# RocketFlash/EmbeddingNet

Hardware: AMD Instinct MI355X
Metric: images/sec training (ResNet18, 224², triplet batch-hard) @ 1/2/4/8 GPU (higher is better)
Workload: dtype f32; 1 GPU; resnet18 224x224x3 synthetic U[0,1), 107-class P x K sampling, local batch 32x4=128 (139 resident batches cycled), E=256, margin 0.5, mining 'hardest' per local batch, radam, fp32 tensors (conv products on 16-bit MFMA from operand splits, fp32 accumulate: 3x3 stride-1 convs and their weight gradients, and the ResNets' other convs where both operands' ranges are known: two fp16 pieces + a per-tenso; global_batch=128, parallelism=dp1, active_triplets_min=192, dead_steps=0, resident_batches=139, step_mode=eager, mining=hardest

## Files before the change

### embeddingnet_amd/csrc/conv_patch.hip

```cpp
#include "gemm_engine.h"
#include "conv_geom.h"
#include "multi_tensor.h"
#include "../../include/embnet.h"

namespace embnet {
namespace patch {

typedef __attribute__((address_space(3))) void* lds_ptr;
__device__ __forceinline__ void dma16(__amdgpu_buffer_rsrc_t r, unsigned char* lds, unsigned voff, unsigned soff) {
  __builtin_amdgcn_raw_ptr_buffer_load_lds(r, (lds_ptr)lds, 16, (int)voff, (int)soff, 0, 0);
}

template <int BN_>
struct GeomP {
  static constexpr int BM = 256, BN = BN_, WAVES_M = 4, WAVES_N = 2, WTM = 64, WTN = BN_ / 2, TM = 2, TN = WTN / 32;
};

struct PatchParams {
  const unsigned short* xp;
  const unsigned short* wp;
  float* y; const float* bias; const float* residual; float* stats; int stats_rows; int relu;
  ConvGeom g; unsigned x_plane_bytes, w_plane_bytes;
  int PH, PW; FastDiv dPHW, dPW;
  int LR;
  int n_full, parts, cc_part, n_pieces, grid; float* ws;
  BnSums bn;
  const uint32_t* a_range; unsigned x32_bytes;
};

typedef const PatchParams __attribute__((address_space(4)))* kargp;
__device__ __forceinline__ kargp kargs() {
  kargp pp = (kargp)__builtin_amdgcn_kernarg_segment_ptr();
  asm volatile("" : "+s"(pp));
  return pp;
}

struct Item { int m0, n0, cc_b, cc_e, tile_m; float* part; };

template <int BN, int CCH = 16>
__device__ __forceinline__ Item work_item(int item, int n_mine) {
  kargp pp = kargs();
  const int b = blockIdx.x, NCC = pp->g.C / CCH, tiles_n = (pp->g.K + BN - 1) / BN;
  Item t; int id;
  if (item < n_mine) {
    id = b + item * pp->grid; t.cc_b = 0; t.cc_e = NCC; t.part = nullptr;
  }
  else {
    id = pp->n_full + b / pp->parts;
    t.cc_b = (b % pp->parts) * pp->cc_part; t.cc_e = min(NCC, t.cc_b + pp->cc_part);
    t.part = pp->ws + (long)b * (256 * BN);
  }
  t.tile_m = id / tiles_n; t.m0 = t.tile_m * 256; t.n0 = (id % tiles_n) * BN;
  return t;
}

__device__ __forceinline__ int padded_pos(int m) {
  kargp pp = kargs();
  FastDiv dOHW, dOW;
  dOHW.mul = pp->g.dOHW.mul; dOHW.shift = pp->g.dOHW.shift; dOHW.d = pp->g.dOHW.d;
  dOW.mul = pp->g.dOW.mul; dOW.shift = pp->g.dOW.shift; dOW.d = pp->g.dOW.d;
  uint32_t n, rem, oh, ow;
  dOHW.divmod((uint32_t)m, n, rem); dOW.divmod(rem, oh, ow);
  return (int)n * (pp->PH * pp->PW) + (int)oh * pp->PW + (int)ow;
}

template <class G, bool F16, int NP>
__device__ __forceinline__ void step_planes(const bf16x8 (&a)[G::TM][NP], const bf16x8 (&b)[G::TN][NP], f32x16 (&acc)[G::TM][G::TN]) {
  if constexpr (F16) {
    f16x8 ah[G::TM][2], bh[G::TN][2];
#pragma unroll
    for (int i = 0; i < G::TM; ++i) { ah[i][0] = __builtin_bit_cast(f16x8, a[i][0]); ah[i][1] = __builtin_bit_cast(f16x8, a[i][1]); }
#pragma unroll
    for (int i = 0; i < G::TN; ++i) { bh[i][0] = __builtin_bit_cast(f16x8, b[i][0]); bh[i][1] = __builtin_bit_cast(f16x8, b[i][1]); }
    mfma_step_h<G::TM, G::TN>(ah, bh, acc);
  } else {
    mfma_step3<G>(a, b, acc);
  }
}

template <class G, int BN, bool BNS, bool F16>
__device__ __forceinline__ void patch_epilogue(const PatchParams& p, const Item& cur, f32x16 (&acc)[G::TM][G::TN], int M, int K,
                                               int wave, int lane, int h, int wm, int wn) {
  constexpr int TM = G::TM, TN = G::TN;
  if (F16) {
    const float osx = p.a_range ? scale_pair(scale_exponent_of(__uint_as_float(*p.a_range))).y
                                : planes_scale_slot(p.xp, (long)(p.x_plane_bytes >> 1))[1];
    const float osw = planes_scale_slot(p.wp, (long)(p.w_plane_bytes >> 1))[1];
#pragma unroll
    for (int im = 0; im < TM; ++im)
#pragma unroll
      for (int in = 0; in < TN; ++in)
#pragma unroll
        for (int rr = 0; rr < 16; ++rr) acc[im][in][rr] = (acc[im][in][rr] * osw) * osx;
  }
  if (cur.part) {
    float* part = cur.part + (wm + 4 * h) * BN + wn + (lane & 31);
#pragma unroll
    for (int im = 0; im < TM; ++im)
#pragma unroll
      for (int in = 0; in < TN; ++in)
#pragma unroll
        for (int rr = 0; rr < 16; ++rr)
          part[(im * 32 + (rr & 3) + 8 * (rr >> 2)) * BN + in * 32] = acc[im][in][rr];
  } else {
    const bool inner = cur.m0 + 256 <= M && cur.n0 + BN <= K;
#pragma unroll
// ... 31 lines not shown
#pragma unroll
          for (int rr = 0; rr < 16; ++rr) {
            p.y[o0 + (long)((rr & 3) + 8 * (rr >> 2)) * K] = v[rr];
            if (BNS) {
              const float e = ev[BNS ? im : 0][rr], dz = act_grad(p.bn.act, fmaf(e, bsc, bsh), v[rr]);
              s1 += dz; s2 = fmaf(dz, (e - bmu) * brs, s2);
            } else { s1 += v[rr]; s2 = fmaf(v[rr], v[rr], s2); }
          }
        } else {
#pragma unroll
          for (int rr = 0; rr < 16; ++rr) {
            const int row = cur.m0 + wm + im * 32 + (rr & 3) + 8 * (rr >> 2) + 4 * h;
            if (row < M && cok) {
              const long o = o0 + (long)((rr & 3) + 8 * (rr >> 2)) * K;
              if (p.residual) v[rr] += p.residual[o];
              p.y[o] = v[rr];
              if (BNS) {
                const float e = ev[BNS ? im : 0][rr], dz = act_grad(p.bn.act, fmaf(e, bsc, bsh), v[rr]);
                s1 += dz; s2 = fmaf(dz, (e - bmu) * brs, s2);
              } else { s1 += v[rr]; s2 = fmaf(v[rr], v[rr], s2); }
            }
          }
        }
      }
      if (p.stats || bnm) {
        s1 += __shfl_xor(s1, 32, 64); s2 += __shfl_xor(s2, 32, 64);
        if (h == 0 && cok) {
          float* const dst = bnm ? p.bn.partial : p.stats;
          const long prow = (long)cur.tile_m * G::WAVES_M + wave / G::WAVES_N, P = bnm ? p.bn.rows : p.stats_rows;
          dst[(long)col * P + prow] = s1;
          dst[((long)K + col) * P + prow] = s2;
        }
      }
    }
  }

}

template <int BN, int R, int S, int TPS, int NBS, bool BNS = false, bool F16 = false, bool PIPE = false>
__global__ __launch_bounds__(640) void conv_patch_kernel(const PatchParams p) {
  using G = GeomP<BN>;
  constexpr int NP = F16 ? 2 : 3;
  constexpr int TM = G::TM, TN = G::TN, SPC = R * S / TPS, D = NBS - 1;
  constexpr int SBY = TPS * NP * BN * 32;
  constexpr int NBI = TPS * NP * (BN / 32);
  static_assert((R * S) % TPS == 0 && SPC >= 2, "steps per chunk");
  extern __shared__ __attribute__((aligned(16))) unsigned char smem[];
  const int tid = threadIdx.x, lane = tid & 63, h = lane >> 5;
  const int wave = __builtin_amdgcn_readfirstlane(tid >> 6);
  const int LR = p.LR, PLP = LR * 32, PB = NP * PLP;
  unsigned char* const bslot0 = smem + 2 * PB;
  const int b = blockIdx.x;
  const int n_mine = b < p.n_full ? (p.n_full - b + p.grid - 1) / p.grid : 0;
  const int n_items = n_mine + (b < p.n_pieces ? 1 : 0);
  if (n_items == 0) return;
  const int dhalf = (lane & 1) ^ ((lane >> 4) & 1);

  if (wave == 8) {
    const __amdgpu_buffer_rsrc_t wr = __builtin_amdgcn_make_buffer_rsrc(const_cast<unsigned short*>(p.wp), 0, 3u * p.w_plane_bytes, 0x00020000);
    const int K = p.g.K, NCC = p.g.C / 16;
    const unsigned wpb = p.w_plane_bytes;
    int it = 0; Item t = work_item<BN>(0, n_mine);
    int cc = t.cc_b, st = 0; bool live = true;
    unsigned rowoff[BN / 32];
    auto tile_rows = [&]() {
#pragma unroll
      for (int gb = 0; gb < BN / 32; ++gb) {
        const int row = t.n0 + gb * 32 + (lane >> 1);
        rowoff[gb] = row < K ? 32u * (unsigned)row + 16u * dhalf : OOB;
      }
    };
    tile_rows();
    auto issue = [&](int gs) {
      unsigned char* slot = bslot0 + (gs % NBS) * SBY;
#pragma unroll
      for (int tp = 0; tp < TPS; ++tp) {
        const int tap = st * TPS + tp, r = tap / S, s = tap % S;
        const unsigned so = 32u * (unsigned)(((r * NCC + cc) * S + s) * K);
#pragma unroll
        for (int q = 0; q < NP; ++q)
#pragma unroll
          for (int gb = 0; gb < BN / 32; ++gb)
            dma16(wr, slot + ((tp * NP + q) * BN + gb * 32) * 32, live ? rowoff[gb] : OOB, q * wpb + so);
      }
      if (live && ++st == SPC) {
        st = 0;
        if (++cc == t.cc_e) {
          if (++it < n_items) { t = work_item<BN>(it, n_mine); cc = t.cc_b; tile_rows(); } else live = false;
        }
      }
    };
    int total = 0;
    for (int i = 0; i < n_items; ++i) { const Item q = work_item<BN>(i, n_mine); total += (q.cc_e - q.cc_b) * SPC; }
    for (int gs = 0; gs < D; ++gs) issue(gs);
    for (int gs = 0; gs < total; ++gs) {
      asm volatile("s_waitcnt vmcnt(%0)" :: "n"((D - 1) * NBI) : "memory");
      __builtin_amdgcn_s_barrier();
      issue(gs + D);
    }
    asm volatile("s_waitcnt vmcnt(0)" ::: "memory");
    return;
  }
  if (wave == 9) {
    const __amdgpu_buffer_rsrc_t xr = __builtin_amdgcn_make_buffer_rsrc(const_cast<unsigned short*>(p.xp), 0, 3u * p.x_plane_bytes, 0x00020000);
    const int NG = LR / 32;
    const unsigned xpb = p.x_plane_bytes, chunk_bytes = 32u * (unsigned)(p.g.N * p.g.H * p.g.W);
    unsigned poff[16];
    auto tile_offsets = [&](const Item& t) {
      kargp pp = kargs();
      FastDiv dPHW, dPW;
      dPHW.mul = pp->dPHW.mul; dPHW.shift = pp->dPHW.shift; dPHW.d = pp->dPHW.d;
      dPW.mul = pp->dPW.mul; dPW.shift = pp->dPW.shift; dPW.d = pp->dPW.d;
      const int P0 = padded_pos(t.m0), N = pp->g.N, H = pp->g.H, W = pp->g.W, pt = pp->g.pad_t, pl = pp->g.pad_l;
#pragma unroll
      for (int gI = 0; gI < 16; ++gI) {
        const int idx = P0 + 32 * gI + (lane >> 1);
        uint32_t n, rem, py, px;
        dPHW.divmod((uint32_t)idx, n, rem); dPW.divmod(rem, py, px);
        const int ih = (int)py - pt, iw = (int)px - pl;
        const bool ok = gI < NG && (int)n < N && (unsigned)ih < (unsigned)H && (unsigned)iw < (unsigned)W;
        poff[gI] = ok ? 32u * (unsigned)(((int)n * H + ih) * W + iw) + 16u * dhalf : OOB;
      }
    };
    auto issue = [&](int cc, int gc) {
      unsigned char* buf = smem + (gc & 1) * PB;
#pragma unroll
      for (int q = 0; q < NP; ++q)
#pragma unroll
        for (int gI = 0; gI < 16; ++gI)
          if (gI < NG) dma16(xr, buf + q * PLP + gI * 1024, poff[gI], q * xpb + (unsigned)cc * chunk_bytes);
    };
    int it = 0; Item t = work_item<BN>(0, n_mine);
    int cc = t.cc_b; bool live = true;
    tile_offsets(t);
    auto advance = [&]() {
      if (++cc == t.cc_e) {
        if (++it < n_items) { t = work_item<BN>(it, n_mine); cc = t.cc_b; tile_offsets(t); } else live = false;
      }
    };
    issue(cc, 0); advance();
    int total_chunks = 0;
    for (int i = 0; i < n_items; ++i) { const Item q = work_item<BN>(i, n_mine); total_chunks += q.cc_e - q.cc_b; }
    for (int gc = 0; gc < total_chunks; ++gc) {
      asm volatile("s_waitcnt vmcnt(0)" ::: "memory");
      __builtin_amdgcn_s_barrier();
      if (live) { issue(cc, gc + 1); advance(); }
#pragma unroll 1
      for (int s2 = 1; s2 < SPC; ++s2) __builtin_amdgcn_s_barrier();
    }
    asm volatile("s_waitcnt vmcnt(0)" ::: "memory");
    return;
  }

  const int wm = (wave / G::WAVES_N) * G::WTM, wn = (wave % G::WAVES_N) * G::WTN;
  const int K = p.g.K, PW = p.PW, M = p.g.N * p.g.OH * p.g.OW;
  int gs = 0, gc = 0;
  f32x16 acc[TM][TN];
  for (int item = 0; item < n_items; ++item) {
    const Item cur = work_item<BN>(item, n_mine);
    int rowidx[TM];
    {
      const int P0 = padded_pos(cur.m0);
#pragma unroll
      for (int im = 0; im < TM; ++im) {
        const int m = cur.m0 + wm + im * 32 + (lane & 31);
        rowidx[im] = m < M ? padded_pos(m) - P0 : 0;
      }
    }
#pragma unroll
    for (int i = 0; i < TM; ++i)
#pragma unroll
      for (int j = 0; j < TN; ++j)
#pragma unroll
        for (int r = 0; r < 16; ++r) acc[i][j][r] = 0.f;
    for (int cc = cur.cc_b; cc < cur.cc_e; ++cc) {
      const unsigned char* pbuf = smem + (gc & 1) * PB;
      if constexpr (F16 && PIPE) {
        f16x8 fa[2][TM][2], fb[2][TN][2];
        auto load_a = [&](int tap, f16x8 (&a)[TM][2]) {
          const int r = tap / S, s2 = tap % S;
#pragma unroll
          for (int im = 0; im < TM; ++im) {
            const int idx = rowidx[im] + r * PW + s2;
            const unsigned char* ap = pbuf + idx * 32 + ((h ^ ((idx >> 3) & 1)) << 4);
#pragma unroll
            for (int q = 0; q < 2; ++q) a[im][q] = *reinterpret_cast<const f16x8*>(ap + q * PLP);
          }
        };
        auto load_b = [&](const unsigned char* bs, int tp, f16x8 (&b)[TN][2]) {
#pragma unroll
          for (int in = 0; in < TN; ++in) {
            const int row = wn + in * 32 + (lane & 31);
            const unsigned char* bp = bs + (tp * 2 * BN + row) * 32 + ((h ^ ((row >> 3) & 1)) << 4);
#pragma unroll
            for (int q = 0; q < 2; ++q) b[in][q] = *reinterpret_cast<const f16x8*>(bp + q * BN * 32);
          }
        };
        constexpr int NT = R * S, NRD = 2 * (TM + TN), NMF = 3 * TM * TN;
#pragma unroll
        for (int t = 0; t < NT; ++t) {
          const int tp = t % TPS;
          if (tp == 0) {
            __syncthreads();
            if (t == 0) load_a(0, fa[0]);
            load_b(bslot0 + (gs % NBS) * SBY, 0, fb[t & 1]);
            __builtin_amdgcn_sched_barrier(0);
          }
          const unsigned char* bs = bslot0 + (gs % NBS) * SBY;
          const bool nxt_a = t + 1 < NT, nxt_b = tp + 1 < TPS;
          if (nxt_a) load_a(t + 1, fa[(t + 1) & 1]);
          if (nxt_b) load_b(bs, tp + 1, fb[(t + 1) & 1]);
          mfma_step_h<TM, TN>(fa[t & 1], fb[t & 1], acc);
          constexpr int NR_AB = NRD, NR_A = 2 * TM;
          const int nr = (nxt_a ? NR_A : 0) + (nxt_b ? NR_AB - NR_A : 0);
#pragma unroll
          for (int i = 0; i < NMF; ++i) {
            __builtin_amdgcn_sched_group_barrier(0x008, 1, 0);
            if (i < nr) __builtin_amdgcn_sched_group_barrier(0x100, 1, 0);
          }
          __builtin_amdgcn_sched_barrier(0);
          if (tp == TPS - 1) ++gs;
        }
        ++gc;
        continue;
      }
#pragma unroll 1
      for (int st = 0; st < SPC; ++st) {
        __syncthreads();
        const unsigned char* bs = bslot0 + (gs % NBS) * SBY;
#pragma unroll
        for (int tp = 0; tp < TPS; ++tp) {
          const int tap = st * TPS + tp, r = tap / S, s = tap % S;
          bf16x8 a[TM][NP], bb[TN][NP];
#pragma unroll
          for (int im = 0; im < TM; ++im) {
            const int idx = rowidx[im] + r * PW + s;
            const unsigned char* ap = pbuf + idx * 32 + ((h ^ ((idx >> 3) & 1)) << 4);
#pragma unroll
            for (int q = 0; q < NP; ++q) a[im][q] = *reinterpret_cast<const bf16x8*>(ap + q * PLP);
          }
#pragma unroll
          for (int in = 0; in < TN; ++in) {
            const int row = wn + in * 32 + (lane & 31);
            const unsigned char* bp = bs + (tp * NP * BN + row) * 32 + ((h ^ ((row >> 3) & 1)) << 4);
#pragma unroll
            for (int q = 0; q < NP; ++q) bb[in][q] = *reinterpret_cast<const bf16x8*>(bp + q * BN * 32);
          }
          step_planes<G, F16>(a, bb, acc);
          if (TPS > 1) __builtin_amdgcn_sched_barrier(0);
        }
        ++gs;
      }
      ++gc;
    }
    patch_epilogue<G, BN, BNS, F16>(p, cur, acc, M, K, wave, lane, h, wm, wn);
  }
}

template <int BN, int G, int NS, bool F16>
__global__ __launch_bounds__(704) void conv1x1_planes_kernel(const PatchParams p) {
  using GP = GeomP<BN>;
  static_assert(F16, "the 1x1 planes kernel is built for the two-piece fp16 format");
  constexpr int NP = 2, TM = GP::TM, TN = GP::TN, D = NS - 1;
  constexpr int A_BYTES = G * NP * 256 * 32, B_BYTES = G * NP * BN * 32, STAGE = A_BYTES + B_BYTES;
  constexpr int NBI_B = G * NP * (BN / 32), NBI_A = NP * 8;
  extern __shared__ __attribute__((aligned(16))) unsigned char smem[];
  const int tid = threadIdx.x, lane = tid & 63, h = lane >> 5;
  const int wave = __builtin_amdgcn_readfirstlane(tid >> 6);
  const int b = blockIdx.x;
  const int n_mine = b < p.n_full ? (p.n_full - b + p.grid - 1) / p.grid : 0;
  const int n_items = n_mine + (b < p.n_pieces ? 1 : 0);
  if (n_items == 0) return;
  const int dhalf = (lane & 1) ^ ((lane >> 4) & 1);
  int total = 0;
  for (int i = 0; i < n_items; ++i) { const Item q = work_item<BN, 16 * G>(i, n_mine); total += q.cc_e - q.cc_b; }

  if (wave >= 8) {
    const bool is_b = wave == 8;
    const int tp = wave - 9;
    const __amdgpu_buffer_rsrc_t rs = is_b
        ? __builtin_amdgcn_make_buffer_rsrc(const_cast<unsigned short*>(p.wp), 0, 3u * p.w_plane_bytes, 0x00020000)
        : __builtin_amdgcn_make_buffer_rsrc(const_cast<unsigned short*>(p.xp), 0, 3u * p.x_plane_bytes, 0x00020000);
    const int K = p.g.K;
    const unsigned wpb = p.w_plane_bytes, xpb = p.x_plane_bytes, chunk_bytes = 32u * (unsigned)(p.g.N * p.g.H * p.g.W);
    int it = 0; Item t = work_item<BN, 16 * G>(0, n_mine);
    int cg = t.cc_b; bool live = true;
    unsigned off[8];
    auto tile_offsets = [&]() {
      if (is_b) {
#pragma unroll
        for (int gb = 0; gb < BN / 32; ++gb) {
          const int row = t.n0 + gb * 32 + (lane >> 1);
          off[gb] = row < K ? 32u * (unsigned)row + 16u * dhalf : OOB;
        }
      } else {
        kargp pp = kargs();
        FastDiv dOHW, dOW;
        dOHW.mul = pp->g.dOHW.mul; dOHW.shift = pp->g.dOHW.shift; dOHW.d = pp->g.dOHW.d;
        dOW.mul = pp->g.dOW.mul; dOW.shift = pp->g.dOW.shift; dOW.d = pp->g.dOW.d;
        const int M = pp->g.N * pp->g.OH * pp->g.OW, st = pp->g.stride, H = pp->g.H, W = pp->g.W;
#pragma unroll
        for (int gI = 0; gI < 8; ++gI) {
          const int m = t.m0 + 32 * gI + (lane >> 1);
          uint32_t n, rem, oh, ow;
          dOHW.divmod((uint32_t)min(m, M - 1), n, rem); dOW.divmod(rem, oh, ow);
          off[gI] = m < M ? 32u * (unsigned)(((int)n * H + (int)oh * st) * W + (int)ow * st) + 16u * dhalf : OOB;
        }
// ... 317 lines not shown
  const int c4 = C / 4;
  float amax = 0.f;
  const float sc = MODE == 1 ? planes_scale_slot(planes, plane)[0] : 1.f;
  for (long i = (long)blockIdx.x * 256 + threadIdx.x; i < total4; i += (long)gridDim.x * 256) {
    const float4 v = reinterpret_cast<const float4*>(x)[i];
    if (MODE == 2) { amax = fmaxf(amax, fmaxf(fmaxf(fabsf(v.x), fabsf(v.y)), fmaxf(fabsf(v.z), fabsf(v.w)))); continue; }
    const long pix = i / c4; const int c = (int)(i % c4) * 4;
    const Split4H s = split4h(v, sc);
    const long o = ((long)(c >> 4) * pixels + pix) * 16 + (c & 15);
#pragma unroll
    for (int q = 0; q < 2; ++q) *reinterpret_cast<uint2*>(planes + q * plane + o) = s.p[q];
  }
  if (MODE == 2) {
    amax = wave_max(amax);
    __shared__ float wm[4];
    if ((threadIdx.x & 63) == 0) wm[threadIdx.x >> 6] = amax;
    __syncthreads();
    if (threadIdx.x == 0) planes_scale_slot(planes, plane)[2 + blockIdx.x] = fmaxf(fmaxf(wm[0], wm[1]), fmaxf(wm[2], wm[3]));
  }
}
__global__ __launch_bounds__(256) void planes_scale_of_kernel(float* __restrict__ slot, int blocks) {
  float m = 0.f;
  for (int i = threadIdx.x; i < blocks; i += 256) m = fmaxf(m, slot[2 + i]);
  m = wave_max(m);
  __shared__ float wm[4];
  if ((threadIdx.x & 63) == 0) wm[threadIdx.x >> 6] = m;
  __syncthreads();
  if (threadIdx.x == 0) {
    m = fmaxf(fmaxf(wm[0], wm[1]), fmaxf(wm[2], wm[3]));
    const float2 sp = scale_pair(scale_exponent_of(m));
    slot[0] = sp.x; slot[1] = sp.y;
  }
}

}
}

using namespace embnet;
using namespace embnet::patch;

static int patch_rows(int n, int oh, int ow, int r, int s) {
  const long M = (long)n * oh * ow;
  const int PH = oh + r - 1, PW = ow + s - 1;
  auto base = [&](long m) { const long img = m / ((long)oh * ow), rem = m % ((long)oh * ow); return img * PH * PW + (rem / ow) * PW + rem % ow; };
  long worst = 0;
  for (long m0 = 0; m0 < M; m0 += 256) {
    const long m1 = (m0 + 256 < M ? m0 + 256 : M) - 1;
    const long L = base(m1) - base(m0) + (long)(r - 1) * PW + s;
    if (L > worst) worst = L;
  }
  return (int)((worst + 31) / 32 * 32);
}

struct Plan { int bn, tps, nbs, LR, tiles, n_full, parts, cc_part, n_pieces, grid; size_t lds, ws_bytes; };

static void plan_tiles(Plan& pl, long M, int k, int ncc) {
  pl.tiles = cdiv(M, 256) * cdiv(k, pl.bn);
  pl.grid = 256;
  pl.n_full = pl.tiles / pl.grid * pl.grid;
  const int rem = pl.tiles - pl.n_full;
  pl.parts = 1; pl.cc_part = ncc; pl.n_pieces = 0; pl.ws_bytes = 0;
  if (rem > 0) {
    int parts = pl.grid / rem; if (parts > ncc) parts = ncc; if (parts < 1) parts = 1;
    pl.cc_part = cdiv(ncc, parts); pl.parts = cdiv(ncc, pl.cc_part);
    if (pl.parts == 1) { pl.n_full = pl.tiles; }
    else { pl.n_pieces = rem * pl.parts; pl.ws_bytes = (size_t)pl.n_pieces * 256 * pl.bn * 4; }
  }
}

constexpr int ONE_G = 2, ONE_NS = 3;
static bool make_plan1(int n, int c, int k, int stride, int oh, int ow, Plan& pl) {
  pl = Plan{};
  if (!planes_f16() || (stride != 1 && stride != 2) || (c % (16 * ONE_G)) || (k & 3) || n <= 0 || oh <= 0 || ow <= 0) return false;
  const size_t in_pix = (size_t)n * ((size_t)(oh - 1) * stride + 1) * ((size_t)(ow - 1) * stride + 1);
  if (in_pix * 32 >= 0x7FFFFFF0ull || (size_t)n * oh * ow * k * 4 >= 0x7FFFFFF0ull) return false;
  pl.bn = k >= 128 ? 128 : 64;
  pl.tps = ONE_G; pl.nbs = ONE_NS; pl.LR = 256;
  pl.lds = (size_t)ONE_NS * ONE_G * 2 * 32 * (256 + pl.bn);
  plan_tiles(pl, (long)n * oh * ow, k, c / (16 * ONE_G));
  return true;
}

static bool make_plan(int n, int c, int r, int s, int k, int stride, int oh, int ow, Plan& pl) {
  if (r == 1 && s == 1) return make_plan1(n, c, k, stride, oh, ow, pl);
  static const int enabled = (int)env_long("EMBNET_CONV_PATCH", 1);
  if (!enabled || stride != 1 || r != 3 || s != 3 || (c & 15) || (k & 3) || n <= 0 || oh <= 0 || ow <= 0) return false;
  if ((size_t)n * (oh + 2) * (ow + 2) * 32 >= 0x7FFFFFF0ull || (size_t)n * oh * ow * c * 2 >= 0x7FFFFFF0ull / 3) return false;
  struct Key { int n, c, k, oh, ow; };
  static thread_local Key keys[8]; static thread_local Plan plans[8]; static thread_local int used = 0, next = 0;
  for (int i = 0; i < used; ++i)
    if (keys[i].n == n && keys[i].c == c && keys[i].k == k && keys[i].oh == oh && keys[i].ow == ow) { pl = plans[i]; return pl.bn != 0; }
  pl = Plan{};
  const size_t np = planes_f16() ? 2 : 3;
  pl.bn = k >= 128 ? 128 : 64;
  pl.tps = pl.bn == 64 ? 3 : 1;
  pl.nbs = pl.bn == 64 ? 3 : 6;
  pl.LR = patch_rows(n, oh, ow, r, s);
  static const int tps3 = (int)env_long("EMBNET_PATCH_TPS3", planes_f16() ? 1 : 0);
  if (pl.bn == 128 && tps3 && 2 * np * pl.LR * 32 + (size_t)2 * 3 * np * 128 * 32 <= BIG_LDS_BYTES) {
    pl.tps = 3; pl.nbs = 2;
    if (np == 2 && 2 * np * pl.LR * 32 + (size_t)3 * 3 * np * 128 * 32 <= BIG_LDS_BYTES) pl.nbs = 3;
  }
  pl.lds = 2 * np * pl.LR * 32 + (size_t)pl.nbs * pl.tps * np * pl.bn * 32;
  if (pl.bn == 128 && pl.tps == 1 && pl.lds > BIG_LDS_BYTES) {
    pl.nbs = 4;
    pl.lds = 2 * np * pl.LR * 32 + (size_t)pl.nbs * pl.tps * np * pl.bn * 32;
  }
  bool ok = pl.LR <= 512 && pl.lds <= BIG_LDS_BYTES;
  if (ok) plan_tiles(pl, (long)n * oh * ow, k, c / 16);
  else pl.bn = 0;
  keys[next] = Key{n, c, k, oh, ow}; plans[next] = pl; next = (next + 1) % 8; if (used < 8) ++used;
  return ok;
}

extern "C" int embnet_conv2d_patch_supported(int n, int c, int r, int s, int k, int stride, int oh, int ow) {
  Plan pl; return make_plan(n, c, r, s, k, stride, oh, ow, pl) ? 1 : 0;
}
extern "C" size_t embnet_conv2d_patch_workspace_bytes(int n, int c, int r, int s, int k, int oh, int ow) {
  Plan pl; return make_plan(n, c, r, s, k, 1, oh, ow, pl) ? pl.ws_bytes : 0;
}
extern "C" int embnet_conv2d_patch_stats_rows(int n, int oh, int ow) { return cdiv((long)n * oh * ow, 256) * 4; }

extern "C" int embnet_planes_from_f32(const float* x, long pixels, int c, void* planes, void* stream) {
  EMBNET_CHECK_ARG(x && planes && pixels > 0 && c > 0 && (c & 15) == 0, "planes_from_f32: need c %% 16 == 0");
  EMBNET_CHECK_ARG((size_t)pixels * c * 2 < 0x7FFFFFF0ull / 3, "planes_from_f32: tensor too large");
  const long n4 = pixels * c / 4;
  EMBNET_TRACE("embnet::patch::planes_from_f32_kernel", TRACE_BYTES, 10.0 * pixels * c, stream);
  const int blocks = (int)(n4 / 256 + 1 > 4096 ? 4096 : n4 / 256 + 1);
  if (planes_f16()) {
    hipStream_t st = (hipStream_t)stream;
    float* slot = planes_scale_slot(planes, pixels * c);
    const int dry = (int)(2 * n4 - 2 < blocks ? 2 * n4 - 2 : blocks);
    planes16_from_f32_kernel<2><<<dry, 256, 0, st>>>(x, pixels, c, (unsigned short*)planes);
    planes_scale_of_kernel<<<1, 256, 0, st>>>(slot, dry);
    planes16_from_f32_kernel<1><<<blocks, 256, 0, st>>>(x, pixels, c, (unsigned short*)planes);
    return check_launch("planes_from_f32");
  }
  planes_from_f32_kernel<<<blocks, 256, 0, (hipStream_t)stream>>>(x, pixels, c, (unsigned short*)planes);
  return check_launch("planes_from_f32");
}

extern "C" int embnet_conv_weight_planes_chunk_elems(void) { return MT_CHUNK; }
extern "C" int embnet_conv_weight_planes(const void* table, int n_tensors, const int32_t* chunks, int n_chunks, void* stream) {
  EMBNET_CHECK_ARG(table && chunks && n_tensors > 0 && n_chunks > 0, "conv_weight_planes: bad argument");
  EMBNET_TRACE("embnet::patch::weight_planes_kernel", TRACE_BYTES, 10.0 * MT_CHUNK * n_chunks, stream);
  if (planes_f16()) {
    hipStream_t st = (hipStream_t)stream;
    weight_scale_kernel<<<cdiv(n_tensors, 256), 256, 0, st>>>((const WPlanesTensor*)table, n_tensors, 0);
    weight_absmax_kernel<<<n_chunks, 256, 0, st>>>((const WPlanesTensor*)table, chunks);
    weight_scale_kernel<<<cdiv(n_tensors, 256), 256, 0, st>>>((const WPlanesTensor*)table, n_tensors, 1);
    weight_planes_kernel<<<n_chunks, 256, 0, st>>>((const WPlanesTensor*)table, chunks, 1);
    return check_launch("conv_weight_planes");
  }
  weight_planes_kernel<<<n_chunks, 256, 0, (hipStream_t)stream>>>((const WPlanesTensor*)table, chunks, 0);
  return check_launch("conv_weight_planes");
}

template <auto Kernel>
static void launch_planes(const PatchParams& p, int threads, size_t lds, hipStream_t st) {
  allow_big_lds<Kernel>();
  Kernel<<<p.grid, threads, lds, st>>>(p);
}
typedef void (*PlanesLaunch)(const PatchParams& p, const Plan& pl, hipStream_t st);

static int launch_planes_gemm(PatchParams& p, Plan pl, const char* kname, double operand_bytes, PlanesLaunch launch,
                              void* workspace, size_t workspace_bytes, void* stream, const char* who) {
  const ConvGeom& g = p.g;
  const long M = (long)g.N * g.OH * g.OW;
  p.stats_rows = cdiv(M, 256) * 4;
  p.grid = pl.grid;
  if (pl.n_pieces > 0 && (pl.ws_bytes > workspace_bytes || !workspace)) { pl.n_full = pl.tiles; pl.n_pieces = 0; pl.parts = 1; }
  p.n_full = pl.n_full; p.parts = pl.parts; p.cc_part = pl.cc_part; p.n_pieces = pl.n_pieces; p.ws = (float*)workspace;
  hipStream_t st = (hipStream_t)stream;
  {
    EMBNET_TRACE_FLOP(kname, 2.0 * M * g.K * g.R * g.S * g.C, operand_bytes + 4.0 * (double)M * g.K * (p.residual ? 2 : 1), st);
    launch(p, pl, st);
  }
  if (p.n_pieces > 0)
    launch_tail_fixup(p.ws, p.parts, 256, pl.bn, 64, p.n_full, pl.tiles - p.n_full, cdiv(g.K, pl.bn), M, g.K, p.bias, p.relu, p.residual,
                      p.y, p.stats, p.stats_rows, p.bn, st);
  return check_launch(who);
}

template <int BN, int TPS, int NBS>
static void launch_patch_as(const PatchParams& p, size_t lds, hipStream_t st) {
  if (!p.bn.x) {
    if (planes_f16()) launch_planes<conv_patch_kernel<BN, 3, 3, TPS, NBS, false, true, true>>(p, 640, lds, st);
    else launch_planes<conv_patch_kernel<BN, 3, 3, TPS, NBS, false, false>>(p, 640, lds, st);
  } else if (!planes_f16()) launch_planes<conv_patch_kernel<BN, 3, 3, TPS, NBS, true, false>>(p, 640, lds, st);
  else launch_planes<conv_patch_kernel<BN, 3, 3, TPS, NBS, true, true>>(p, 640, lds, st);
}
static void launch_patch(const PatchParams& p, const Plan& pl, hipStream_t st) {
  if (pl.bn == 128 && pl.tps == 3) { if (pl.nbs == 3) launch_patch_as<128, 3, 3>(p, pl.lds, st); else launch_patch_as<128, 3, 2>(p, pl.lds, st); }
  else if (pl.bn == 128) { if (pl.nbs == 6) launch_patch_as<128, 1, 6>(p, pl.lds, st); else launch_patch_as<128, 1, 4>(p, pl.lds, st); }
  else launch_patch_as<64, 3, 3>(p, pl.lds, st);
}

static int conv2d_patch_impl(const void* xp, const void* wp, const float* bias, float* y, int n, int h, int wd, int c,
                             int r, int s, int k, int pad_t, int pad_l, int oh, int ow, int relu,
                             const float* residual, float* stats, const BnSums& bsum, void* workspace, size_t workspace_bytes,
                             void* stream) {
  EMBNET_CHECK_ARG(xp && wp && y, "conv2d_patch: null pointer");
  EMBNET_CHECK_ARG(r == 3 && s == 3, "conv2d_patch: 3x3 kernels (1x1: embnet_conv2d_planes1x1_f32)");
  Plan pl;
  EMBNET_CHECK_ARG(make_plan(n, c, r, s, k, 1, oh, ow, pl), "conv2d_patch: unsupported geometry (see embnet_conv2d_patch_supported)");
  PatchParams p{(const unsigned short*)xp, (const unsigned short*)wp, y, bias, residual, stats, 0, relu};
  if (int rc = make_geom(p.g, n, h, wd, c, r, s, k, 1, pad_t, pad_l, oh, ow, "conv2d_patch")) return rc;
  p.x_plane_bytes = (unsigned)((size_t)n * h * wd * c * 2);
  p.w_plane_bytes = (unsigned)((size_t)r * s * c * k * 2);
  p.PH = oh + r - 1; p.PW = ow + s - 1;
  p.dPHW = FastDiv::make(p.PH * p.PW); p.dPW = FastDiv::make(p.PW);
  p.LR = pl.LR;
  p.bn = bsum;
  static thread_local char kname[160];
  snprintf(kname, sizeof kname, "void embnet::patch::conv_patch_kernel<%d, 3, 3, %d, %d, %s%s>(embnet::patch::PatchParams)", pl.bn, pl.tps, pl.nbs,
           p.bn.x ? "true" : "false", planes_f16() ? (p.bn.x ? ", true" : ", true, true") : "");
  return launch_planes_gemm(p, pl, kname, (planes_f16() ? 4.0 : 6.0) * ((double)n * h * wd * c + (double)r * s * c * k), launch_patch,
                            workspace, workspace_bytes, stream, "conv2d_patch");
}

extern "C" int embnet_conv2d_patch_f32(const void* xp, const void* wp, const float* bias, float* y, int n, int h, int wd, int c,
                                       int r, int s, int k, int pad_t, int pad_l, int oh, int ow, int relu,
                                       const float* residual, float* stats, void* workspace, size_t workspace_bytes,
                                       void* stream) {
  return conv2d_patch_impl(xp, wp, bias, y, n, h, wd, c, r, s, k, pad_t, pad_l, oh, ow, relu, residual, stats, NO_BN_SUMS, workspace,
                           workspace_bytes, stream);
// ... 70 lines not shown
```

### include/embnet.h

```cpp
#ifndef EMBNET_H
#define EMBNET_H

#include <stddef.h>
#include <stdint.h>

#ifdef __cplusplus
extern "C" {
#endif

#define EMBNET_ABI_VERSION 22

enum {
  EMBNET_MINE_SEMIHARD = 0,
  EMBNET_MINE_HARDEST = 1,
  EMBNET_MINE_RANDOM_HARD = 2,
  EMBNET_MINE_BATCH_HARD = 3
};

int embnet_abi_version(void);
const char* embnet_last_error(void);

int embnet_trace_enable(int on);
int embnet_trace_reset(void);
int embnet_trace_count(void);
// ... 112 lines not shown
                                   void* stream);
size_t embnet_conv2d_wgrad_workspace_bytes(int n, int c, int r, int s, int k, int oh, int ow);
int embnet_conv2d_wgrad_f32(const float* x, const float* dy, float* dw, void* workspace, size_t workspace_bytes,
                            int n, int h, int wd, int c, int r, int s, int k, int stride, int pad_t, int pad_l,
                            int oh, int ow, const float* in_scale, const float* in_shift, int in_act, void* stream);

int embnet_conv2d_wgrad_slabs_f32(const float* x, const float* dy, float* dw, void* workspace, size_t workspace_bytes,
                                  int n, int h, int wd, int c, int r, int s, int k, int stride, int pad_t, int pad_l,
                                  int oh, int ow, const float* in_scale, const float* in_shift, int in_act,
                                  void* stream);
int embnet_conv2d_wgrad_reduce_f32(const float* x, const float* dy, float* dw, void* workspace, size_t workspace_bytes,
                                   int n, int h, int wd, int c, int r, int s, int k, int stride, int pad_t, int pad_l,
                                   int oh, int ow, const float* in_scale, const float* in_shift, int in_act,
                                   void* stream);
int embnet_conv2d_wgrad_splits(int n, int c, int r, int s, int k, int oh, int ow);
int embnet_slab_reduce_multi(const void* host_table, int n_tensors, void* stream);

int embnet_range_from_bound(const float* bound, int c, float factor, const uint32_t* add_range, uint32_t* out, void* stream);
int embnet_range_slot_words(void);
int embnet_range_emit(uint32_t* slot);
int embnet_range_chunk_elems(void);
int embnet_range_multi(const void* table, int n_tensors, const int32_t* chunks, int n_chunks, void* stream);
int embnet_conv2d_ranges(const uint32_t* a, const uint32_t* b);
int embnet_conv2d_fwd_f32_ex(const float* x, const float* w, const float* bias, float* y, int n, int h, int wd, int c,
                             int r, int s, int k, int stride, int pad_t, int pad_l, int oh, int ow, int relu,
                             const float* residual, const float* in_scale, const float* in_shift, int in_act,
                             float* stats, void* workspace, size_t workspace_bytes, const uint32_t* x_range,
                             const uint32_t* w_range, void* stream);
int embnet_conv2d_dgrad_f32_ex(const float* dy, const float* w, float* dx, int n, int h, int wd, int c, int r, int s,
                               int k, int stride, int pad_t, int pad_l, int oh, int ow, int accumulate, const float* dx_add,
                               void* workspace, size_t workspace_bytes, const uint32_t* dy_range, const uint32_t* w_range,
                               void* stream);
int embnet_conv2d_dgrad_bnsums_f32_ex(const float* dy, const float* w, float* dx, int n, int h, int wd, int c, int r, int s,
                                      int k, int stride, int pad_t, int pad_l, int oh, int ow, const float* bn_x,
                                      const float* bn_scale, const float* bn_shift, const float* bn_mean, const float* bn_rstd,
                                      int bn_act, float* bn_partial, int bn_rows, void* workspace, size_t workspace_bytes,
                                      const uint32_t* dy_range, const uint32_t* w_range, void* stream);
int embnet_conv2d_wgrad_f32_ex(const float* x, const float* dy, float* dw, void* workspace, size_t workspace_bytes,
                               int n, int h, int wd, int c, int r, int s, int k, int stride, int pad_t, int pad_l,
                               int oh, int ow, const float* in_scale, const float* in_shift, int in_act,
                               const uint32_t* x_range, const uint32_t* dy_range, void* stream);
int embnet_conv2d_wgrad_slabs_f32_ex(const float* x, const float* dy, float* dw, void* workspace, size_t workspace_bytes,
                                     int n, int h, int wd, int c, int r, int s, int k, int stride, int pad_t, int pad_l,
                                     int oh, int ow, const float* in_scale, const float* in_shift, int in_act,
                                     const uint32_t* x_range, const uint32_t* dy_range, void* stream);

const char* embnet_conv2d_kernel_name(int kind, int n, int h, int wd, int c, int r, int s, int k, int oh, int ow);

int embnet_conv1x1_thin_supported(int red, int ncols);

int embnet_conv2d_patch_supported(int n, int c, int r, int s, int k, int stride, int oh, int ow);
size_t embnet_conv2d_patch_workspace_bytes(int n, int c, int r, int s, int k, int oh, int ow);
int embnet_conv2d_patch_stats_rows(int n, int oh, int ow);
int embnet_conv2d_patch_f32(const void* x_planes, const void* w_planes, const float* bias, float* y, int n, int h, int wd, int c,
                            int r, int s, int k, int pad_t, int pad_l, int oh, int ow, int relu, const float* residual,
                            float* stats, void* workspace, size_t workspace_bytes, void* stream);
int embnet_conv2d_stem_supported(int n, int h, int wd, int c, int r, int s, int k, int stride, int pad_t, int pad_l, int oh, int ow);
int embnet_conv2d_stem_stats_rows(int n, int oh, int ow);
int embnet_conv2d_stem_f32(const float* x, const float* w, float* y, int n, int h, int wd, int pad_t, int pad_l, int oh, int ow,
                           float* stats, const uint32_t* x_range, const uint32_t* w_range, void* stream);
int embnet_conv2d_planes1x1_f32(const void* x_planes, const void* w_planes, const float* bias, float* y, int n, int h, int wd, int c,
                                int k, int stride, int oh, int ow, int relu, const float* residual, float* stats,
                                void* workspace, size_t workspace_bytes, void* stream);
int embnet_conv2d_dma1x1_supported(int n, int h, int wd, int c, int k, int stride, int oh, int ow);
int embnet_conv2d_dma1x1_f32(const float* x, const void* wp, const float* bias, float* y, int n, int h, int wd, int c, int k,
                             int stride, int oh, int ow, int relu, const float* residual, float* stats, const uint32_t* x_range,
                             void* workspace, size_t workspace_bytes, void* stream);
int embnet_conv2d_patch_bnsums_f32(const void* x_planes, const void* w_planes, float* y, int n, int h, int wd, int c, int r, int s,
                                   int k, int pad_t, int pad_l, int oh, int ow, const float* bn_x, const float* bn_scale,
                                   const float* bn_shift, const float* bn_mean, const float* bn_rstd, int bn_act,
                                   float* bn_partial, int bn_rows, void* workspace, size_t workspace_bytes, void* stream);
int embnet_se_mlp_supported(int n, int c, int s);
int embnet_se_mlp_fwd(const float* pooled, const float* w1, const float* b1, const float* w2, const float* b2, int n, int c, int s,
                      float* z1, float* gate, void* stream);
int embnet_se_mlp_bwd(const float* dgate, const float* gate, const float* z1, const float* pooled, const float* w1, const float* w2,
                      int n, int c, int s, float* dz1, float* dpooled, float* dw1, float* db1, float* dw2, float* db2, void* stream);
int embnet_planes_from_f32(const float* x, long pixels, int c, void* planes, void* stream);
int embnet_conv_weight_planes_chunk_elems(void);
int embnet_conv_weight_planes(const void* table, int n_tensors, const int32_t* chunks, int n_chunks, void* stream);
int embnet_affine_act_planes(const float* x, long m, int c, const float* scale, const float* shift, int act, float* y,
                             void* planes, void* stream);
int embnet_affine_act_planes_ex(const float* x, long m, int c, const float* scale, const float* shift, int act, float* y,
                                void* planes, const float* y_bound, uint32_t* y_range, void* stream);
int embnet_conv2d_wgrad_planes_supported(int n, int h, int wd, int c, int r, int s, int k, int stride, int pad_t, int pad_l,
                                         int oh, int ow);
int embnet_conv2d_wgrad_planes_splits(int n, int h, int wd, int c, int k);
size_t embnet_conv2d_wgrad_planes_workspace_bytes(int n, int h, int wd, int c, int k);
int embnet_conv2d_wgrad_planes_f32(const void* x_planes, const void* dy_planes, float* dw, void* workspace,
                                   size_t workspace_bytes, int n, int h, int wd, int c, int k, int reduce, void* stream);

int embnet_u8_to_f32(const void* src, const int32_t* index, int n, long pixels, int c_in, int c_out, float denom, float* dst,
                     void* stream);

size_t embnet_augment_param_floats(void);
int embnet_augment_params(const float* ops, int n_ops, uint64_t seed, uint64_t batch_no, int n, int h, int w, float* table,
                          void* stream);
int embnet_augment_apply(const void* src, const int32_t* index, int n, int h, int w, int c_in, int c_out, const float* table,
                         uint64_t seed, uint64_t batch_no, float* dst, void* stream);
int embnet_augment_params_clahe(const float* ops, int n_ops, const float* clahe_rec, int clahe_pos, uint64_t seed,
                                uint64_t batch_no, int n, int h, int w, float* table, void* stream);
size_t embnet_augment_clahe_lut_bytes(int n, int gx, int gy);
int embnet_augment_clahe_luts(const void* src, const int32_t* index, int n, int h, int w, int c_in, int gx, int gy,
                              const float* table, void* luts, void* stream);
int embnet_augment_apply_clahe(const void* src, const int32_t* index, int n, int h, int w, int c_in, int c_out, const float* table,
                               const void* luts, int gx, int gy, uint64_t seed, uint64_t batch_no, float* dst, void* stream);

// ... 305 lines not shown
```

Baseline: 16850 images/sec.

## Balance patch-conv tail tiles with stream-K splits and ticket-based combine

Replaces the old fixed split of leftover tiles into equal channel-chunk parts with a stream-K style tail. The remaining tile-by-channel-chunk units are spread evenly across a fixed 256-workgroup grid. Workgroups that share a tile write partial accumulators to workspace slots, and the last one to arrive (per-wave atomic ticket) sums them and runs the epilogue. This targets wave-quantization imbalance in the last round of tiles. It adds global atomics, workspace traffic, per-stream ticket sets and a host-side planner that only applies the cut when the estimated span improves.

Measured after the change: 16310 images/sec. -3.2%, worse.

```diff
diff --git a/embeddingnet_amd/csrc/conv_patch.hip b/embeddingnet_amd/csrc/conv_patch.hip
--- a/embeddingnet_amd/csrc/conv_patch.hip
+++ b/embeddingnet_amd/csrc/conv_patch.hip
@@ -1,7 +1,10 @@
 #include "gemm_engine.h"
 #include "conv_geom.h"
 #include "multi_tensor.h"
+#include "patch_plan.h"
 #include "../../include/embnet.h"
+#include <mutex>
+#include <string.h>
 
 namespace embnet {
 namespace patch {
@@ -24,6 +27,8 @@
   int PH, PW; FastDiv dPHW, dPW;
   int LR;
   int n_full, parts, cc_part, n_pieces, grid; float* ws;
+  int tail_q, tail_r, ticket_set;
+  unsigned short tail_slot0[TAIL_GRID];
   BnSums bn;
   const uint32_t* a_range; unsigned x32_bytes;
 };
@@ -35,7 +40,10 @@
   return pp;
 }
 
-struct Item { int m0, n0, cc_b, cc_e, tile_m; float* part; };
+struct Item {
+  int m0, n0, cc_b, cc_e, tile_m; float* part;
+  int np, idx, slot0, tail_tile;
+};
 
 template <int BN, int CCH = 16>
 __device__ __forceinline__ Item work_item(int item, int n_mine) {
@@ -52,6 +60,73 @@
   }
   t.tile_m = id / tiles_n; t.m0 = t.tile_m * 256; t.n0 = (id % tiles_n) * BN;
   return t;
+}
+
+template <int BN>
+__device__ __forceinline__ Item patch_item(int item, int n_mine) {
+  kargp pp = kargs();
+  const int b = blockIdx.x, NCC = pp->g.C / 16, tiles_n = (pp->g.K + BN - 1) / BN;
+  Item t; int id;
+  t.part = nullptr; t.np = 1; t.idx = 0; t.slot0 = 0; t.tail_tile = 0;
+  if (item < n_mine) { id = b + item * pp->grid; t.cc_b = 0; t.cc_e = NCC; }
+  else {
+    const TailItem ti = tail_item(NCC, pp->tail_q, pp->tail_r, b, item - n_mine);
+    id = pp->n_full + ti.tile; t.cc_b = ti.cc_b; t.cc_e = ti.cc_e;
+    t.np = ti.np; t.idx = ti.idx; t.tail_tile = ti.tile; t.slot0 = pp->tail_slot0[ti.tile];
+  }
+  t.tile_m = id / tiles_n; t.m0 = t.tile_m * 256; t.n0 = (id % tiles_n) * BN;
+  return t;
+}
+
+constexpr int TICKET_SETS = 16;
+__device__ unsigned g_tail_ticket[TICKET_SETS][TAIL_GRID * TAIL_WAVES];
+
+template <class G, int BN>
+__device__ __forceinline__ bool tail_combine(const PatchParams& p, const Item& cur, f32x16 (&acc)[G::TM][G::TN], int wave, int lane) {
+  constexpr int TM = G::TM, TN = G::TN, SLOT_BYTES = 256 * BN * 4;
+  const unsigned mine = (unsigned)((wave * TM * TN * 4) * 64 + lane) * 16u;
+  const uint64_t sa = reinterpret_cast<uint64_t>(p.ws + (long)cur.slot0 * (256 * BN));
+  float* const slots = reinterpret_cast<float*>((uint64_t)(uint32_t)__builtin_amdgcn_readfirstlane((int)(uint32_t)sa) |
+                                                ((uint64_t)(uint32_t)__builtin_amdgcn_readfirstlane((int)(uint32_t)(sa >> 32)) << 32));
+  const __amdgpu_buffer_rsrc_t sr = __builtin_amdgcn_make_buffer_rsrc(slots, 0, cur.np * SLOT_BYTES, 0x00020000);
+  typedef uint32_t u32x4 __attribute__((ext_vector_type(4)));
+#pragma unroll
+  for (int im = 0; im < TM; ++im)
+#pragma unroll
+    for (int in = 0; in < TN; ++in)
+#pragma unroll
+      for (int q = 0; q < 4; ++q) {
+        const float4 v = make_float4(acc[im][in][4 * q], acc[im][in][4 * q + 1], acc[im][in][4 * q + 2], acc[im][in][4 * q + 3]);
+        __builtin_amdgcn_raw_buffer_store_b128(__builtin_bit_cast(u32x4, v), sr, mine + (unsigned)(((im * TN + in) * 4 + q) * 64 * 16),
+                                               cur.idx * SLOT_BYTES, 16);
+      }
+  asm volatile("s_waitcnt vmcnt(0)" ::: "memory");
+  unsigned* const ticket = &g_tail_ticket[p.ticket_set][cur.tail_tile * TAIL_WAVES + wave];
+  unsigned old = 0;
+  if (lane == 0) old = __hip_atomic_fetch_add(ticket, 1u, __ATOMIC_RELAXED, __HIP_MEMORY_SCOPE_AGENT);
+  old = (unsigned)__builtin_amdgcn_readfirstlane((int)old);
+  if ((int)old != cur.np - 1) return false;
+  __builtin_amdgcn_fence(__ATOMIC_ACQUIRE, "agent");
+  asm volatile("s_waitcnt vmcnt(0)" ::: "memory");
+  if (lane == 0) __hip_atomic_store(ticket, 0u, __ATOMIC_RELAXED, __HIP_MEMORY_SCOPE_AGENT);
+
+  auto piece = [&](int j, int blk, int q) {
+    const u32x4 v = __builtin_amdgcn_raw_buffer_load_b128(sr, mine + (unsigned)((blk * 4 + q) * 64 * 16), j * SLOT_BYTES, 16);
+    return __builtin_bit_cast(float4, v);
+  };
+  for (int j = 0; j < cur.np; ++j) {
+#pragma unroll
+    for (int im = 0; im < TM; ++im)
+#pragma unroll
+      for (int in = 0; in < TN; ++in)
+#pragma unroll
+        for (int q = 0; q < 4; ++q) {
+          const float4 v = piece(j, im * TN + in, q);
+          if (j == 0) { acc[im][in][4 * q] = v.x; acc[im][in][4 * q + 1] = v.y; acc[im][in][4 * q + 2] = v.z; acc[im][in][4 * q + 3] = v.w; }
+          else { acc[im][in][4 * q] += v.x; acc[im][in][4 * q + 1] += v.y; acc[im][in][4 * q + 2] += v.z; acc[im][in][4 * q + 3] += v.w; }
+        }
+  }
+  return true;
 }
 
 __device__ __forceinline__ int padded_pos(int m) {
@@ -189,7 +264,7 @@
   unsigned char* const bslot0 = smem + 2 * PB;
   const int b = blockIdx.x;
   const int n_mine = b < p.n_full ? (p.n_full - b + p.grid - 1) / p.grid : 0;
-  const int n_items = n_mine + (b < p.n_pieces ? 1 : 0);
+  const int n_items = n_mine + tail_item_count(p.g.C / 16, p.tail_q, p.tail_r, b);
   if (n_items == 0) return;
   const int dhalf = (lane & 1) ^ ((lane >> 4) & 1);
 
@@ -197,7 +272,7 @@
     const __amdgpu_buffer_rsrc_t wr = __builtin_amdgcn_make_buffer_rsrc(const_cast<unsigned short*>(p.wp), 0, 3u * p.w_plane_bytes, 0x00020000);
     const int K = p.g.K, NCC = p.g.C / 16;
     const unsigned wpb = p.w_plane_bytes;
-    int it = 0; Item t = work_item<BN>(0, n_mine);
+    int it = 0; Item t = patch_item<BN>(0, n_mine);
     int cc = t.cc_b, st = 0; bool live = true;
     unsigned rowoff[BN / 32];
     auto tile_rows = [&]() {
@@ -223,12 +298,12 @@
       if (live && ++st == SPC) {
         st = 0;
         if (++cc == t.cc_e) {
-          if (++it < n_items) { t = work_item<BN>(it, n_mine); cc = t.cc_b; tile_rows(); } else live = false;
+          if (++it < n_items) { t = patch_item<BN>(it, n_mine); cc = t.cc_b; tile_rows(); } else live = false;
         }
       }
     };
     int total = 0;
-    for (int i = 0; i < n_items; ++i) { const Item q = work_item<BN>(i, n_mine); total += (q.cc_e - q.cc_b) * SPC; }
+    for (int i = 0; i < n_items; ++i) { const Item q = patch_item<BN>(i, n_mine); total += (q.cc_e - q.cc_b) * SPC; }
     for (int gs = 0; gs < D; ++gs) issue(gs);
     for (int gs = 0; gs < total; ++gs) {
       asm volatile("s_waitcnt vmcnt(%0)" :: "n"((D - 1) * NBI) : "memory");
@@ -267,17 +342,17 @@
         for (int gI = 0; gI < 16; ++gI)
           if (gI < NG) dma16(xr, buf + q * PLP + gI * 1024, poff[gI], q * xpb + (unsigned)cc * chunk_bytes);
     };
-    int it = 0; Item t = work_item<BN>(0, n_mine);
+    int it = 0; Item t = patch_item<BN>(0, n_mine);
     int cc = t.cc_b; bool live = true;
     tile_offsets(t);
     auto advance = [&]() {
       if (++cc == t.cc_e) {
-        if (++it < n_items) { t = work_item<BN>(it, n_mine); cc = t.cc_b; tile_offsets(t); } else live = false;
+        if (++it < n_items) { t = patch_item<BN>(it, n_mine); cc = t.cc_b; tile_offsets(t); } else live = false;
       }
     };
     issue(cc, 0); advance();
     int total_chunks = 0;
-    for (int i = 0; i < n_items; ++i) { const Item q = work_item<BN>(i, n_mine); total_chunks += q.cc_e - q.cc_b; }
+    for (int i = 0; i < n_items; ++i) { const Item q = patch_item<BN>(i, n_mine); total_chunks += q.cc_e - q.cc_b; }
     for (int gc = 0; gc < total_chunks; ++gc) {
       asm volatile("s_waitcnt vmcnt(0)" ::: "memory");
       __builtin_amdgcn_s_barrier();
@@ -294,7 +369,7 @@
   int gs = 0, gc = 0;
   f32x16 acc[TM][TN];
   for (int item = 0; item < n_items; ++item) {
-    const Item cur = work_item<BN>(item, n_mine);
+    const Item cur = patch_item<BN>(item, n_mine);
     int rowidx[TM];
     {
       const int P0 = padded_pos(cur.m0);
@@ -390,6 +465,7 @@
       }
       ++gc;
     }
+    if (cur.np > 1 && !tail_combine<G, BN>(p, cur, acc, wave, lane)) continue;
     patch_epilogue<G, BN, BNS, F16>(p, cur, acc, M, K, wave, lane, h, wm, wn);
   }
 }
@@ -813,7 +889,16 @@
   return (int)((worst + 31) / 32 * 32);
 }
 
-struct Plan { int bn, tps, nbs, LR, tiles, n_full, parts, cc_part, n_pieces, grid; size_t lds, ws_bytes; };
+struct Plan { int bn, tps, nbs, LR, tiles, n_full, parts, cc_part, n_pieces, grid; size_t lds, ws_bytes; TailPlan tail; };
+
+static void plan_patch_tiles(Plan& pl, long M, int k, int ncc) {
+  pl.tiles = cdiv(M, 256) * cdiv(k, pl.bn);
+  pl.grid = TAIL_GRID;
+  plan_tail(pl.tail, pl.tiles, ncc);
+  pl.n_full = pl.tail.n_full;
+  pl.parts = 1; pl.cc_part = ncc; pl.n_pieces = 0;
+  pl.ws_bytes = (size_t)pl.tail.n_slots * 256 * pl.bn * 4;
+}
 
 static void plan_tiles(Plan& pl, long M, int k, int ncc) {
   pl.tiles = cdiv(M, 256) * cdiv(k, pl.bn);
@@ -868,7 +953,7 @@
     pl.lds = 2 * np * pl.LR * 32 + (size_t)pl.nbs * pl.tps * np * pl.bn * 32;
   }
   bool ok = pl.LR <= 512 && pl.lds <= BIG_LDS_BYTES;
-  if (ok) plan_tiles(pl, (long)n * oh * ow, k, c / 16);
+  if (ok) plan_patch_tiles(pl, (long)n * oh * ow, k, c / 16);
   else pl.bn = 0;
   keys[next] = Key{n, c, k, oh, ow}; plans[next] = pl; next = (next + 1) % 8; if (used < 8) ++used;
   return ok;
@@ -881,6 +966,30 @@
   Plan pl; return make_plan(n, c, r, s, k, 1, oh, ow, pl) ? pl.ws_bytes : 0;
 }
 extern "C" int embnet_conv2d_patch_stats_rows(int n, int oh, int ow) { return cdiv((long)n * oh * ow, 256) * 4; }
+
+static bool tail_plan_of(long m, int c, int k, TailPlan& tp) {
+  if (m <= 0 || c < 16 || (c & 15) || k <= 0 || cdiv(m, 256) * (long)cdiv(k, 64) > 0x7FFFFFFF) return false;
+  plan_tail(tp, (int)(cdiv(m, 256) * cdiv(k, k >= 128 ? 128 : 64)), c / 16);
+  return true;
+}
+extern "C" int embnet_conv2d_patch_tail_plan(long m, int c, int k, int32_t* out) {
+  TailPlan tp;
+  EMBNET_CHECK_ARG(out && tail_plan_of(m, c, k, tp), "conv2d_patch_tail_plan: m > 0, c %% 16 == 0, k > 0");
+  const int32_t v[12] = {tp.tiles, tp.ncc, tp.n_full, tp.rem, tp.units, tp.q, tp.r, tp.n_slots, tp.cut, tp.span, tp.span_whole, tp.span_today};
+  for (int i = 0; i < 12; ++i) out[i] = v[i];
+  return 0;
+}
+extern "C" int embnet_conv2d_patch_tail_items(long m, int c, int k, int workgroup, int32_t* out, int max_items) {
+  TailPlan tp;
+  EMBNET_CHECK_ARG(out && tail_plan_of(m, c, k, tp) && workgroup >= 0 && workgroup < TAIL_GRID, "conv2d_patch_tail_items: bad argument");
+  const int n = tp.cut ? tail_item_count(tp.ncc, tp.q, tp.r, workgroup) : 0;
+  for (int j = 0; j < n && j < max_items; ++j) {
+    const TailItem t = tail_item(tp.ncc, tp.q, tp.r, workgroup, j);
+    const int32_t v[6] = {t.tile, t.cc_b, t.cc_e, t.np, t.idx, t.np > 1 ? tp.slot0[t.tile] + t.idx : -1};
+    for (int i = 0; i < 6; ++i) out[6 * j + i] = v[i];
+  }
+  return n;
+}
 
 extern "C" int embnet_planes_from_f32(const float* x, long pixels, int c, void* planes, void* stream) {
   EMBNET_CHECK_ARG(x && planes && pixels > 0 && c > 0 && (c & 15) == 0, "planes_from_f32: need c %% 16 == 0");
@@ -924,6 +1033,15 @@
 }
 typedef void (*PlanesLaunch)(const PatchParams& p, const Plan& pl, hipStream_t st);
 
+static int ticket_set_of(hipStream_t st) {
+  static std::mutex mu; static hipStream_t owner[TICKET_SETS]; static int used = 0;
+  std::lock_guard<std::mutex> lock(mu);
+  for (int i = 0; i < used; ++i) if (owner[i] == st) return i;
+  if (used == TICKET_SETS) return -1;
+  owner[used] = st;
+  return used++;
+}
+
 static int launch_planes_gemm(PatchParams& p, Plan pl, const char* kname, double operand_bytes, PlanesLaunch launch,
                               void* workspace, size_t workspace_bytes, void* stream, const char* who) {
   const ConvGeom& g = p.g;
@@ -931,8 +1049,17 @@
   p.stats_rows = cdiv(M, 256) * 4;
   p.grid = pl.grid;
   if (pl.n_pieces > 0 && (pl.ws_bytes > workspace_bytes || !workspace)) { pl.n_full = pl.tiles; pl.n_pieces = 0; pl.parts = 1; }
+  hipStream_t st = (hipStream_t)stream;
+  p.tail_q = p.tail_r = p.ticket_set = 0;
+  if (pl.tail.cut) {
+    const int set = pl.ws_bytes > workspace_bytes || !workspace ? -1 : ticket_set_of(st);
+    if (set < 0) pl.n_full = pl.tiles;
+    else {
+      p.tail_q = pl.tail.q; p.tail_r = pl.tail.r; p.ticket_set = set;
+      memcpy(p.tail_slot0, pl.tail.slot0, sizeof p.tail_slot0);
+    }
+  }
   p.n_full = pl.n_full; p.parts = pl.parts; p.cc_part = pl.cc_part; p.n_pieces = pl.n_pieces; p.ws = (float*)workspace;
-  hipStream_t st = (hipStream_t)stream;
   {
     EMBNET_TRACE_FLOP(kname, 2.0 * M * g.K * g.R * g.S * g.C, operand_bytes + 4.0 * (double)M * g.K * (p.residual ? 2 : 1), st);
     launch(p, pl, st);
diff --git a/embeddingnet_amd/csrc/patch_plan.h b/embeddingnet_amd/csrc/patch_plan.h
--- /dev/null
+++ b/embeddingnet_amd/csrc/patch_plan.h
@@ -0,0 +1,78 @@
+#pragma once
+#include <stdint.h>
+
+#if defined(__HIPCC__)
+#define PLAN_HD __host__ __device__ __forceinline__
+#else
+#define PLAN_HD inline
+#endif
+
+namespace embnet {
+namespace patch {
+
+constexpr int TAIL_GRID = 256;
+constexpr int TAIL_WAVES = 8;
+
+constexpr double TAIL_COMBINE_CHUNKS = 0.75;
+
+struct TailItem { int tile, cc_b, cc_e, np, idx; };
+
+PLAN_HD int tail_first_unit(int q, int r, int b) { return b * q + (b < r ? b : r); }
+PLAN_HD int tail_owner(int q, int r, int u) {
+  const int big = r * (q + 1);
+  return u < big ? u / (q + 1) : r + (u - big) / q;
+}
+PLAN_HD int tail_item_count(int ncc, int q, int r, int b) {
+  const int u0 = tail_first_unit(q, r, b), u1 = u0 + q + (b < r ? 1 : 0);
+  return u1 > u0 ? (u1 - 1) / ncc - u0 / ncc + 1 : 0;
+}
+PLAN_HD TailItem tail_item(int ncc, int q, int r, int b, int j) {
+  const int u0 = tail_first_unit(q, r, b), u1 = u0 + q + (b < r ? 1 : 0);
+  TailItem t;
+  t.tile = u0 / ncc + j;
+  const int lo = t.tile * ncc, hi = lo + ncc;
+  t.cc_b = (u0 > lo ? u0 : lo) - lo;
+  t.cc_e = (u1 < hi ? u1 : hi) - lo;
+  const int first = tail_owner(q, r, lo);
+  t.np = tail_owner(q, r, hi - 1) - first + 1;
+  t.idx = b - first;
+  return t;
+}
+
+struct TailPlan {
+  int tiles, ncc, n_full, rem;
+  int units, q, r;
+  int n_slots, cut;
+  int span_whole, span_cut, span_today, span;
+  unsigned short slot0[TAIL_GRID];
+};
+
+inline void plan_tail(TailPlan& tp, int tiles, int ncc) {
+  tp = TailPlan{};
+  tp.tiles = tiles; tp.ncc = ncc;
+  const int rounds = tiles / TAIL_GRID, rem = tiles - rounds * TAIL_GRID;
+  tp.rem = rem; tp.n_full = tiles;
+  tp.span_whole = (rounds + (rem > 0 ? 1 : 0)) * ncc;
+  tp.span_cut = tp.span_today = tp.span = tp.span_whole;
+  if (rem == 0) return;
+  {
+    int parts = TAIL_GRID / rem; if (parts > ncc) parts = ncc;
+    tp.span_today = rounds * ncc + (ncc + parts - 1) / parts;
+  }
+  const int U = rem * ncc;
+  tp.span_cut = rounds * ncc + (U + TAIL_GRID - 1) / TAIL_GRID;
+  if (!(tp.span_cut + TAIL_COMBINE_CHUNKS < tp.span_whole)) return;
+  tp.cut = 1; tp.span = tp.span_cut;
+  tp.n_full = rounds * TAIL_GRID;
+  tp.units = U; tp.q = U / TAIL_GRID; tp.r = U % TAIL_GRID;
+  int slots = 0;
+  for (int t = 0; t < rem; ++t) {
+    const int np = tail_owner(tp.q, tp.r, (t + 1) * ncc - 1) - tail_owner(tp.q, tp.r, t * ncc) + 1;
+    tp.slot0[t] = (unsigned short)slots;
+    if (np > 1) slots += np;
+  }
+  tp.n_slots = slots;
+}
+
+}
+}
diff --git a/include/embnet.h b/include/embnet.h
--- a/include/embnet.h
+++ b/include/embnet.h
@@ -188,6 +188,8 @@
 int embnet_conv2d_patch_supported(int n, int c, int r, int s, int k, int stride, int oh, int ow);
 size_t embnet_conv2d_patch_workspace_bytes(int n, int c, int r, int s, int k, int oh, int ow);
 int embnet_conv2d_patch_stats_rows(int n, int oh, int ow);
+int embnet_conv2d_patch_tail_plan(long m, int c, int k, int32_t* out);
+int embnet_conv2d_patch_tail_items(long m, int c, int k, int workgroup, int32_t* out, int max_items);
 int embnet_conv2d_patch_f32(const void* x_planes, const void* w_planes, const float* bias, float* y, int n, int h, int wd, int c,
                             int r, int s, int k, int pad_t, int pad_l, int oh, int ow, int relu, const float* residual,
                             float* stats, void* workspace, size_t workspace_bytes, void* stream);
```
